# ohsnyt/bzip2-rust

Hardware: AMD Instinct MI355X
Metric: compress MB/s at -9 (900 KB blocks), 1/2/4/8 MI355X; bit-exact vs C bzip2 (higher is better)
Workload: dtype u8; 1 GPU; 1024 MiB per GPU synthetic text at -9 (1194 blocks on this rank), BASELINE configs[2]; raw_bytes_total=1073741824, blocks_rank0=1194, compressed_bytes=323302688

## Files before the change

bzip2-rust_amd/csrc/bzx_bsort.hip:

```cpp
#include <hip/hip_runtime.h>
#include "bzx_host.h"
#include "bzx_wg.h"
#include "bzx_pack.h"

#define BS_NT 1024
#define BS_NW (BS_NT / 64)
#ifndef BS_C
#define BS_C 2048
#endif
#define BS_FW (BS_C / 64)
#define BS_ISO (BS_C / 3)
#ifndef BS_ISO_SHIFT
#define BS_ISO_SHIFT 5
#endif
#ifndef BS_BIN1
#define BS_BIN1 15
#endif
#define BS_BIN2 12
#define BS_NBIN1 (1u << BS_BIN1)
#define BS_TAB_WORDS (BS_NBIN1 + (BS_NBIN1 >> 5))
#define BS_MAX_BK 1024
#ifndef BS_MAX_BIG
#define BS_MAX_BIG 512
#endif
#define SP_U 4
#ifndef BS_MAX_DEPTH
#define BS_MAX_DEPTH 511
#endif
#ifndef BS_MAX_SPLITS
#define BS_MAX_SPLITS 1024
#endif
#ifndef BS_ROUNDS
#define BS_ROUNDS 4
#endif
#ifndef BS_KEYBITS
#define BS_KEYBITS 32
#endif
#define BS_TINY 64
#define BS_MED 512
#define REC_IDX(r) ((uint32_t)((r) >> 12) & 0xFFFFFu)
#define REC_PREV(r) ((uint32_t)((r) >> 4) & 0xFFu)
#define W_POS_MASK 0x3FFFull

static_assert(BS_C <= 16384, "bucket capacity");

#ifdef BZX_DIAG
__shared__ unsigned long long s_diag[128];
#define DIAG_T0()                                                             \
    unsigned long long t_last_ = 0;                                           \
    if (B.dbg && threadIdx.x == 0) {                                          \
        for (int i_ = 0; i_ < 128; i_++) s_diag[i_] = 0;                      \
        t_last_ = wall_clock64();                                             \
    }                                                                         \
    (void)t_last_;
#define DIAG_STAMP(slot)                                                      \
    do {                                                                      \
        if (B.dbg && threadIdx.x == 0) {                                      \
            const unsigned long long now_ = wall_clock64();                   \
            s_diag[slot] += now_ - t_last_;                                   \
            t_last_ = now_;                                                   \
        }                                                                     \
    } while (0)
#define DIAG_COUNT(slot, v)                                                   \
    do {                                                                      \
        if (B.dbg && threadIdx.x == 0) s_diag[slot] += (unsigned long long)(v); \
    } while (0)
#define DIAG_FLUSH()                                                          \
    do {                                                                      \
        if (B.dbg && threadIdx.x == 0)                                        \
            for (int i_ = 0; i_ < 128; i_++)                                  \
                if (s_diag[i_]) atomicAdd(&B.dbg[i_], s_diag[i_]);            \
    } while (0)
#else
#define DIAG_T0() do {} while (0)
#define DIAG_STAMP(slot) do {} while (0)
#define DIAG_COUNT(slot, v) do {} while (0)
#define DIAG_FLUSH() do {} while (0)
#endif

__shared__ uint32_t b_tab[BS_TAB_WORDS + BS_MAX_BK];
__shared__ uint32_t b_start[BS_MAX_BK + 1];
__shared__ uint32_t b_first[BS_MAX_BK + 1];
__shared__ uint32_t b_cur[BS_MAX_BK];
__shared__ uint8_t b_b0[BS_MAX_BK];
__shared__ uint32_t b_inuse[256];
__shared__ uint8_t b_seq[256];
__shared__ uint32_t b_scratch[2 * BS_NW];
__shared__ uint32_t b_lbase[8];
__shared__ uint32_t b_bcast[12];
__shared__ uint32_t b_big[BS_MAX_BIG][3];

#define TAB(b) b_tab[(b) + ((b) >> 5)]

template <int ISO, int PER>
__device__ __forceinline__ void bucket_flags(const uint32_t (&c)[PER], uint32_t bin0, uint32_t excl, uint32_t prevc, uint32_t &fl, uint32_t &nf)
{
    constexpr uint32_t CP = BS_C - ISO;
    uint32_t s = excl, ps = excl - prevc, pc = prevc;
#pragma unroll
    for (int k = 0; k < PER; k++) {
        const bool f = (bin0 + k == 0) || c[k] > (uint32_t)ISO || pc > (uint32_t)ISO || (s / CP != ps / CP);
        fl |= (uint32_t)f << k;
        nf += f;
        ps = s;
        s += c[k];
        pc = c[k];
    }
}

template <int BINS, bool TAB16 = false>
__device__ __forceinline__ uint32_t form_buckets(uint32_t total)
{
    constexpr int PER = BINS / BS_NT;
    const uint32_t tid = threadIdx.x, bin0 = tid * PER;
    uint32_t c[PER], sum = 0, e8 = 0, e6 = 0, e4 = 0;
#pragma unroll
    for (int k = 0; k < PER; k++) {
        c[k] = TAB(bin0 + k);
        sum += c[k];
        const uint32_t m = c[k] <= BS_ISO ? c[k] : 0u;
        e8 += m > BS_C / 8 ? m : 0u;
        e6 += m > BS_C / 6 ? m : 0u;
        e4 += m > BS_C / 4 ? m : 0u;
    }
    const uint32_t prevc = tid ? TAB(bin0 - 1) : 0u;
    if (__any(e8 != 0)) {
        e8 = bzx_wave_incl_sum(e8);
        e6 = bzx_wave_incl_sum(e6);
        e4 = bzx_wave_incl_sum(e4);
        if (bzx_lane() == 63) {
            atomicAdd(&b_bcast[8], e8);
            if (e6) atomicAdd(&b_bcast[9], e6);
            if (e4) atomicAdd(&b_bcast[10], e4);
        }
    }
    uint32_t tot;
    const uint32_t excl = bzx_block_excl_sum<BS_NT>(sum, b_scratch, tot);
    const uint32_t allow = total >> BS_ISO_SHIFT;
    uint32_t fl = 0, nf = 0;
    if (b_bcast[8] <= allow) bucket_flags<BS_C / 8>(c, bin0, excl, prevc, fl, nf);
    else if (b_bcast[9] <= allow) bucket_flags<BS_C / 6>(c, bin0, excl, prevc, fl, nf);
    else if (b_bcast[10] <= allow) bucket_flags<BS_C / 4>(c, bin0, excl, prevc, fl, nf);
    else bucket_flags<BS_ISO>(c, bin0, excl, prevc, fl, nf);
    uint32_t nbk;
    const uint32_t fexcl = bzx_block_excl_sum<BS_NT>(nf, b_scratch, nbk);
    if (nbk > BS_MAX_BK) return 0;
    {
        uint32_t id = fexcl, s = excl;
#pragma unroll
        for (int k = 0; k < PER; k++) {
            if ((fl >> k) & 1u) {
                b_start[id] = s;
                b_first[id] = bin0 + k;
                id++;
            }
            if (TAB16) reinterpret_cast<uint16_t *>(b_tab)[bin0 + k] = (uint16_t)(id - 1);
            else TAB(bin0 + k) = id - 1;
            s += c[k];
        }
    }
    if (tid == 0) {
        b_start[nbk] = total;
        b_first[nbk] = BINS;
    }
    __syncthreads();
    return nbk;
}

template <int BINW>
__device__ __forceinline__ void bucket_setup(uint32_t nbk)
{
    for (uint32_t k = threadIdx.x; k < nbk; k += BS_NT) {
        const uint32_t first = b_first[k], last = b_first[k + 1] - 1u;
        b_b0[k] = (uint8_t)(first == last ? BINW : (uint32_t)__builtin_clz(first ^ last) - (32u - BINW));
        b_cur[k] = 0;
    }
}

template <int BINW>
__device__ __forceinline__ bool bucket_emit(const BzxBatch &B, uint32_t blk, uint32_t jj, uint32_t nbk, uint32_t base, uint32_t buf,
                                            uint32_t depth, uint32_t bits, uint32_t done, uint32_t salt)
{
    const uint32_t tid = threadIdx.x, cap8 = B.bk_cap >> 3;
    if (!B.bk_affine) jj += salt;
    if (tid < 8) {
        const uint32_t mine = B.bk_affine ? (tid == (jj & 7u) ? nbk : 0u) : (nbk + 7u - ((tid - jj) & 7u)) >> 3;
        uint32_t at = mine ? atomicAdd(&B.counters[BZX_CTR_BK_LIST0 + tid], mine) : 0u;
        if (at + mine > cap8) {
            b_bcast[4] = 1;
            at = 0;
        }
        b_lbase[tid] = tid * cap8 + at;
    }
    __syncthreads();
    if (b_bcast[4]) return false;
    for (uint32_t k = tid; k < nbk; k += BS_NT) {
        BzxBucket it;
        it.blk = blk;
        it.start = (base + b_start[k]) | (buf << 31);
        it.cnt = b_start[k + 1] - b_start[k];
        it.dbits = (depth + b_b0[k]) | (bits << 16);
        if (it.cnt > BS_C) {
            const uint32_t q = atomicAdd(&b_bcast[3], 1u);
            if (q - done < BS_MAX_BIG) {
                b_big[q % BS_MAX_BIG][0] = it.start;
                b_big[q % BS_MAX_BIG][1] = it.cnt;
                b_big[q % BS_MAX_BIG][2] = depth + BINW;
            } else {
                b_bcast[4] = 1;
            }
            it.cnt = 0;
        }
        B.bk_list[B.bk_affine ? b_lbase[jj & 7u] + k : b_lbase[(jj + k) & 7u] + (k >> 3)] = it;
    }
    __syncthreads();
    return b_bcast[4] == 0;
}

struct BzxDeepItem {
    uint32_t blk, st, cnt, dbits;
};

__device__ __forceinline__ uint32_t *rank_array(const BzxBatch &B, uint32_t k, uint32_t which)
{
    if (k >= B.rk_blocks) return nullptr;
    return B.isa2 + ((size_t)k * 2 + which) * BZX_MAX_N;
}

__device__ __forceinline__ void emit_giant(const BzxBatch &B, uint32_t blk, uint64_t *rec_a, const uint64_t *rec_b,
                                           uint32_t st, uint32_t cnt, uint32_t depth, uint32_t bits)
{
    const uint32_t tid = threadIdx.x, base = st & 0x7fffffffu;
    const uint64_t *src = ((st >> 31) ? rec_b : rec_a) + base;
    uint32_t *__restrict__ isa0 = rank_array(B, (uint32_t)BZX_SLAB(B, blk), 0), *__restrict__ isa1 = rank_array(B, (uint32_t)BZX_SLAB(B, blk), 1);
    if (tid == 0) b_bcast[7] = isa0 ? atomicAdd(&B.counters[BZX_CTR_GIANT_CNT], 1u) : 0xFFFFFFFFu;
    __syncthreads();
    const uint32_t at = b_bcast[7];
    const bool listed = at < B.deep_cap;
    for (uint32_t i = tid; i < cnt; i += BS_NT) {
        const uint64_t r = src[i];
        rec_a[base + i] = (uint64_t)REC_IDX(r) | (i == 0 ? 1ull << 32 : 0ull);
        if (isa0) isa0[REC_IDX(r)] = isa1[REC_IDX(r)] = base | (listed ? 0u : RK_COARSE);
    }
    if (tid == 0) {
        atomicMin(&B.blk[blk].n_mtf, depth / bits);
        if (listed) {
            BzxDeepItem it;
            it.blk = blk;
            it.st = base;
            it.cnt = cnt;
            it.dbits = 0;
            reinterpret_cast<BzxDeepItem *>(B.deep_list)[(size_t)2 * B.deep_cap + at] = it;
        }
        atomicAdd(&B.blk[blk].n_groups, 1u);
        if ((atomicOr(&B.blk[blk].status, BZX_ST_RESUME) & BZX_ST_RESUME) == 0)
            B.resume_list[atomicAdd(&B.counters[BZX_CTR_RESUME], 1u)] = blk;
    }
    __syncthreads();
}

__device__ __forceinline__ void block_redo(const BzxBatch &B, uint32_t b)
{
    if ((atomicOr(&B.blk[b].status, BZX_ST_REDO) & BZX_ST_REDO) == 0)
        B.redo_list[atomicAdd(&B.counters[BZX_CTR_REDO], 1u)] = b;
}


__device__ bool deep_process(const BzxBatch &B, uint32_t b, uint32_t j_, uint32_t n, uint32_t bits, const uint8_t *__restrict__ P,
                             uint64_t *__restrict__ rec_a, uint64_t *__restrict__ rec_b, uint32_t done, uint32_t flush_from,
                             int push_lvl)
{
    const uint32_t tid = threadIdx.x;
    bool ok = true;
    while (ok) {
        const uint32_t nbig = b_bcast[3];
        __syncthreads();
        if (done >= nbig) break;
        if (push_lvl >= 0 && done >= flush_from) {
            const uint32_t np = nbig - done;
            if (tid == 0) b_bcast[5] = atomicAdd(&B.counters[BZX_CTR_DEEP_CNT + push_lvl], np);
            __syncthreads();
            const uint32_t at = b_bcast[5];
            __syncthreads();
            if (at + np <= B.deep_cap) {
                BzxDeepItem *dl = reinterpret_cast<BzxDeepItem *>(B.deep_list) + (size_t)(push_lvl & 1) * B.deep_cap + at;
                for (uint32_t q = tid; q < np; q += BS_NT) {
                    const uint32_t r = (done + q) % BS_MAX_BIG;
                    BzxDeepItem it;
                    it.blk = b;
                    it.st = b_big[r][0];
                    it.cnt = b_big[r][1];
                    it.dbits = b_big[r][2] | (bits << 16);
                    dl[q] = it;
                }
                __syncthreads();
                break;
            }
            push_lvl = -1;
        }
        const uint32_t st = b_big[done % BS_MAX_BIG][0], cnt = b_big[done % BS_MAX_BIG][1], depth = b_big[done % BS_MAX_BIG][2];
        done++;
        if (tid == 0) b_bcast[6] = atomicAdd(reinterpret_cast<uint32_t *>(&B.blk[b].pack_word), 1u);
        __syncthreads();
        const uint32_t spent = b_bcast[6];
        const uint32_t base = st & 0x7fffffffu, buf = st >> 31;
        const uint64_t *__restrict__ src = (buf ? rec_b : rec_a) + base;
        uint64_t *__restrict__ dst = (buf ? rec_a : rec_b) + base;
        if (depth + BS_BIN2 + 32 >= n * bits) {
            ok = false;
            break;
        }
        if (depth + BS_BIN2 > BS_MAX_DEPTH || spent >= BS_MAX_SPLITS) {
            emit_giant(B, b, rec_a, rec_b, st, cnt, depth, bits);
            continue;
        }
        constexpr uint32_t NB2 = 1u << BS_BIN2;
        for (uint32_t i = tid; i < NB2 + (NB2 >> 5); i += BS_NT) b_tab[i] = 0;
        if (tid == 0) b_bcast[1] = 0;
        if (tid < 3) b_bcast[8 + tid] = 0;
        __syncthreads();
        for (uint32_t i = tid; i < cnt; i += BS_NT) atomicAdd(&TAB((uint32_t)(src[i] >> (64 - BS_BIN2))), 1u);
        __syncthreads();
        const uint32_t nbk = form_buckets<(int)NB2>(cnt);
        if (nbk == 0) {
            ok = false;
            break;
        }
        bucket_setup<BS_BIN2>(nbk);
        __syncthreads();
        for (uint32_t i = tid; i < cnt; i += BS_NT) {
            const uint64_t r = src[i];
            const uint32_t k = TAB((uint32_t)(r >> (64 - BS_BIN2)));
            uint32_t x = REC_IDX(r) * bits + depth + b_b0[k];
            if (x >= n * bits) x -= n * bits;
            const uint32_t key = (uint32_t)(pk_window_bit(P, x) >> 32);
            const uint32_t slot = atomicAdd(&b_cur[k], 1u);
            dst[b_start[k] + slot] = ((uint64_t)key << 32) | (r & 0xFFFFFFFFull);
        }
        __syncthreads();
        ok = bucket_emit<BS_BIN2>(B, b, j_, nbk, base, buf ^ 1u, depth, bits, done, spent + 1u);
        DIAG_COUNT(104, 1);
        DIAG_COUNT(105, cnt);
    }
    return ok;
}

__global__ __launch_bounds__(BS_NT) void bzx_bsplit_kernel(BzxBatch B)
{
    const uint32_t tid = threadIdx.x;
    DIAG_T0();
    for (;;) {
        if (tid == 0) b_bcast[0] = atomicAdd(&B.counters[BZX_CTR_SPLIT_FETCH], 1u);
        __syncthreads();
        const uint32_t j_ = b_bcast[0];
        __syncthreads();
        if (j_ >= B.nblk) break;
        const uint32_t b = B.blk_first + j_ * B.blk_step;
        const uint32_t n = B.blk[b].n;
        const uint8_t *__restrict__ T = BZX_BLOCK_PTR(B, B.blk[b]);
        const size_t sb = BZX_SLAB(B, b);
        uint8_t *__restrict__ P = B.pk + sb * BZX_PK_STRIDE;
        uint64_t *__restrict__ rec_a = B.rec_a + sb * BZX_MAX_N;
        uint64_t *__restrict__ rec_b = B.rec_b + sb * BZX_MAX_N;

        DIAG_STAMP(96);
        if (tid < 256) b_inuse[tid] = 0;
        if (tid == 0) {
            b_bcast[1] = 0;
            b_bcast[3] = 0;
            b_bcast[4] = 0;
            b_bcast[8] = b_bcast[9] = b_bcast[10] = 0;
            B.blk[b].pack_word = 0;
            B.blk[b].n_mtf = 0xFFFFFFFFu;
            B.blk[b].n_groups = 0;
            B.blk[b].n_selectors = (uint32_t)BZX_SLAB(B, b);
        }
        __syncthreads();
        {
            const uint32_t n16 = n & ~15u;
            for (uint32_t i = tid * 16; i < n16; i += BS_NT * 16) {
                uint4 v;
                __builtin_memcpy(&v, T + i, 16);
                const uint32_t w[4] = {v.x, v.y, v.z, v.w};
#pragma unroll
                for (int q = 0; q < 4; q++)
#pragma unroll
                    for (int k = 0; k < 4; k++) b_inuse[(w[q] >> (8 * k)) & 255u] = 1;
            }
            for (uint32_t i = n16 + tid; i < n; i += BS_NT) b_inuse[T[i]] = 1;
        }
        __syncthreads();
        uint32_t n_in_use;
        {
            const uint32_t flag = tid < 256 ? b_inuse[tid] : 0u;
            const uint32_t ex = bzx_block_excl_sum<BS_NT>(flag, b_scratch, n_in_use);
            if (tid < 256) b_seq[tid] = (uint8_t)ex;
        }
        __syncthreads();
        uint32_t bits = 1;
        while ((1u << bits) < n_in_use) bits++;
        DIAG_STAMP(97);
        pk_build_t<BS_NT>(T, n, bits, P, b_seq);
        DIAG_STAMP(98);

        for (uint32_t i = tid; i < BS_TAB_WORDS; i += BS_NT) b_tab[i] = 0;
        __syncthreads();
        for (uint32_t t0 = 0; t0 < n; t0 += BS_NT * 4 * SP_U) {
            uint64_t x[SP_U];
#pragma unroll
            for (uint32_t u = 0; u < SP_U; u++) {
                const uint32_t i0 = t0 + (u * BS_NT + tid) * 4;
                x[u] = i0 < n ? pk_window(P, i0, bits) : 0ull;
            }
#pragma unroll
            for (uint32_t u = 0; u < SP_U; u++) {
                const uint32_t i0 = t0 + (u * BS_NT + tid) * 4;
#pragma unroll
                for (uint32_t e = 0; e < 4; e++)
                    if (i0 + e < n) atomicAdd(&TAB((uint32_t)((x[u] << (e * bits)) >> (64 - BS_BIN1))), 1u);
            }
        }
        __syncthreads();
        DIAG_STAMP(99);
        uint32_t nbk = form_buckets<(int)BS_NBIN1, true>(n);
        if (nbk) bucket_setup<BS_BIN1>(nbk);
        __syncthreads();
        DIAG_STAMP(100);
        if (nbk == 0) {
            DIAG_COUNT(106, 1);
            if (tid == 0) block_redo(B, b);
            __syncthreads();
            continue;
        }

        {
            constexpr uint32_t SP_TILE = 8192, SP_V = SP_TILE / (BS_NT * 4);
            static_assert(BS_MAX_BK <= BS_NT && BS_TAB_WORDS >= 32768 + BS_MAX_BK, "tile scan: one bucket per lane");
            uint16_t *tab16 = reinterpret_cast<uint16_t *>(b_tab);
            for (uint32_t i = tid; i < BS_NBIN1 / 2; i += BS_NT) {
                uint32_t v = reinterpret_cast<uint32_t *>(b_tab)[i];
                v |= ((uint32_t)b_b0[v & 1023u] << 10) | ((uint32_t)b_b0[(v >> 16) & 1023u] << 26);
                reinterpret_cast<uint32_t *>(b_tab)[i] = v;
            }
            uint64_t *stage = reinterpret_cast<uint64_t *>(b_tab + 16384);
            uint32_t *tcnt0 = b_tab + 32768;
            uint32_t *delta = b_first;
            uint32_t *tcnt1 = tcnt0 + BS_MAX_BK;
            if (tid < nbk) tcnt0[tid] = tcnt1[tid] = 0;
            uint64_t hi[SP_V], lo[SP_V];
            uint32_t pv[SP_V];
            auto load_tile = [&](uint32_t t0) {
#pragma unroll
                for (uint32_t u = 0; u < SP_V; u++) {
                    const uint32_t i0 = t0 + (u * BS_NT + tid) * 4;
                    hi[u] = lo[u] = 0;
                    pv[u] = 0;
                    if (i0 < n) {
                        uint64_t w2[2];
                        __builtin_memcpy(w2, P + ((i0 * bits) >> 3), 16);
                        hi[u] = w2[0];
                        lo[u] = w2[1];
                        if (i0 >= 1 && i0 + 3 <= n) {
                            __builtin_memcpy(&pv[u], T + i0 - 1, 4);
                        } else {
                            const uint32_t nvalid = n - i0 < 4u ? n - i0 : 4u;
                            for (uint32_t e = 0; e < nvalid; e++) pv[u] |= (uint32_t)T[i0 + e ? i0 + e - 1 : n - 1] << (8 * e);
                        }
                    }
                }
            };
            load_tile(0);
            bzx_lds_barrier();
            uint32_t tpar = 0;
            for (uint32_t t0 = 0; t0 < n; t0 += SP_TILE, tpar ^= 1u) {
                uint32_t *tcnt = tpar ? tcnt1 : tcnt0, *tother = tpar ? tcnt0 : tcnt1;
                uint32_t kr[SP_V * 4], key[SP_V * 4], pvc[SP_V];
#pragma unroll
                for (uint32_t u = 0; u < SP_V; u++) {
                    const uint32_t i0 = t0 + (u * BS_NT + tid) * 4;
                    const uint32_t nvalid = i0 < n ? (n - i0 < 4u ? n - i0 : 4u) : 0u;
                    const uint32_t sh0 = (i0 * bits) & 7u;
                    const uint64_t h = __builtin_bswap64(hi[u]), l = __builtin_bswap64(lo[u]);
                    pvc[u] = pv[u];
#pragma unroll
                    for (uint32_t e = 0; e < 4; e++) {
                        kr[u * 4 + e] = 0xFFFFFFFFu;
                        key[u * 4 + e] = 0;
                        if (e < nvalid) {
                            const uint32_t sh = sh0 + e * bits;
                            const uint64_t w = sh ? (h << sh) | (l >> (64u - sh)) : h;
                            const uint32_t kb = tab16[(uint32_t)(w >> (64 - BS_BIN1))], k = kb & 1023u;
                            key[u * 4 + e] = (uint32_t)((w << (kb >> 10)) >> 32);
                            kr[u * 4 + e] = k | (atomicAdd(&tcnt[k], 1u) << 16);
                        }
                    }
                }
                if (t0 + SP_TILE < n) load_tile(t0 + SP_TILE);
                bzx_lds_barrier();
                {
                    const uint32_t c = tid < nbk ? tcnt[tid] : 0u;
                    const uint32_t incl = bzx_wave_incl_sum(c);
                    uint32_t *wtot = b_scratch + tpar * BS_NW;
                    if (bzx_lane() == 63) wtot[bzx_wave()] = incl;
                    bzx_lds_barrier();
                    uint32_t pre = 0;
                    const uint32_t wv = bzx_wave();
#pragma unroll
                    for (uint32_t i = 0; i < BS_NW; i++) pre += i < wv ? wtot[i] : 0u;
                    const uint32_t ex = pre + incl - c;
                    if (tid < nbk) {
                        tcnt[tid] = ex;
                        tother[tid] = 0;
                        delta[tid] = b_start[tid] + b_cur[tid] - ex;
                        b_cur[tid] += c;
                    }
                }
                bzx_lds_barrier();
#pragma unroll
                for (uint32_t u = 0; u < SP_V; u++)
#pragma unroll
                    for (uint32_t e = 0; e < 4; e++)
                        if (kr[u * 4 + e] != 0xFFFFFFFFu) {
                            const uint32_t k = kr[u * 4 + e] & 0xFFFFu, rel = (u * BS_NT + tid) * 4 + e;
                            stage[tcnt[k] + (kr[u * 4 + e] >> 16)] = ((uint64_t)key[u * 4 + e] << 32) | ((uint64_t)k << 21) | ((uint64_t)rel << 8) |
                                                                     (uint64_t)((pvc[u] >> (8 * e)) & 255u);
                        }
                bzx_lds_barrier();
                const uint32_t tn = n - t0 < SP_TILE ? n - t0 : SP_TILE;
#pragma unroll
                for (uint32_t u = 0; u < SP_TILE / BS_NT; u++) {
                    const uint32_t i = u * BS_NT + tid;
                    if (i < tn) {
                        const uint64_t r = stage[i];
                        const uint32_t k = (uint32_t)(r >> 21) & 1023u, rel = (uint32_t)(r >> 8) & 8191u;
                        rec_a[delta[k] + i] = (r & 0xFFFFFFFF00000000ull) | ((uint64_t)(t0 + rel) << 12) | ((r & 255ull) << 4);
                    }
                }
            }
        }
        __syncthreads();
        DIAG_STAMP(101);
        bool ok = bucket_emit<BS_BIN1>(B, b, j_, nbk, 0, 0, 0, bits, 0, 0);
        DIAG_STAMP(102);

        if (ok) ok = deep_process(B, b, j_, n, bits, P, rec_a, rec_b, 0, 0, BZX_DEEP_LEVELS > 0 ? 0 : -1);
        DIAG_STAMP(103);
        if (!ok) DIAG_COUNT(107, 1);
        if (!ok && tid == 0) block_redo(B, b);
        __syncthreads();
    }
    DIAG_FLUSH();
}

__global__ __launch_bounds__(BS_NT) void bzx_bsplit_deep_kernel(BzxBatch B)
{
    const uint32_t tid = threadIdx.x, lvl = B.deep_lvl;
    const uint32_t listed = B.counters[BZX_CTR_DEEP_CNT + lvl];
    const uint32_t n_items = listed < B.deep_cap ? listed : B.deep_cap;
    if (n_items == 0) return;
    DIAG_T0();
    const BzxDeepItem *list = reinterpret_cast<const BzxDeepItem *>(B.deep_list) + (size_t)(lvl & 1u) * B.deep_cap;
    for (;;) {
        if (tid == 0) b_bcast[0] = atomicAdd(&B.counters[BZX_CTR_DEEP_FETCH + lvl], 1u);
        __syncthreads();
        const uint32_t i = b_bcast[0];
        __syncthreads();
        if (i >= n_items) break;
        const BzxDeepItem d = list[i];
        if (d.cnt == 0) continue;
        const uint32_t b = d.blk;
        if (__atomic_load_n(&B.blk[b].status, __ATOMIC_RELAXED) & BZX_ST_REDO) continue;
        const uint32_t n = B.blk[b].n, bits = d.dbits >> 16;
        const size_t sb = BZX_SLAB(B, b);
        const uint8_t *__restrict__ P = B.pk + sb * BZX_PK_STRIDE;
        uint64_t *__restrict__ rec_a = B.rec_a + sb * BZX_MAX_N;
        uint64_t *__restrict__ rec_b = B.rec_b + sb * BZX_MAX_N;
        if (tid == 0) {
            b_bcast[3] = 1;
            b_bcast[4] = 0;
            b_big[0][0] = d.st;
            b_big[0][1] = d.cnt;
            b_big[0][2] = d.dbits & 0xFFFFu;
        }
        __syncthreads();
        const bool ok = deep_process(B, b, (b - B.blk_first) / B.blk_step, n, bits, P, rec_a, rec_b, 0, 1,
                                     lvl + 1 < BZX_DEEP_LEVELS ? (int)lvl + 1 : -1);
        if (!ok && tid == 0) block_redo(B, b);
        __syncthreads();
    }
    DIAG_FLUSH();
}

#ifndef SK_NT
#define SK_NT 256
#endif
#define SK_NW (SK_NT / 64)
#define BS_E (BS_C / SK_NT)
#define SK_DB 8
#define SK_ND (1u << SK_DB)
static_assert(BS_C % SK_NT == 0 && BS_E >= 1 && BS_E <= 8, "bucket capacity");

__shared__ uint64_t s_x[BS_C];
__shared__ __attribute__((aligned(16))) uint64_t s_w[BS_C + 4];
__shared__ __attribute__((aligned(16))) uint32_t s_cnt[SK_NW][SK_ND];
__shared__ uint32_t s_dbase[SK_ND];
__shared__ uint32_t s_part[4];
__shared__ uint64_t s_f[BS_FW + 1];
__shared__ uint32_t s_med[BS_C / BS_TINY + 1];
__shared__ uint32_t s_large[BS_C / BS_MED + 1];
__shared__ uint32_t s_rc[2][4];
__shared__ uint32_t s_bc[8];
__shared__ uint32_t s_m[2];
__shared__ uint32_t s_red[SK_NW][4];

__device__ __forceinline__ uint32_t uni(uint32_t v) { return bzx_uni(v); }
__device__ __forceinline__ uint32_t tid_here() { return bzx_tid_here(); }
__device__ __forceinline__ BzxBucket uni(BzxBucket b)
{
    BzxBucket r;
    r.blk = uni(b.blk);
    r.start = uni(b.start);
    r.cnt = uni(b.cnt);
    if (r.cnt >> 31) r.cnt = 0;
    r.dbits = uni(b.dbits);
    return r;
}

__device__ __forceinline__ void wave_rank(uint32_t *wc, uint32_t d, bool valid, uint32_t lane, uint32_t &old, uint32_t &rank)
{
    uint64_t m = __ballot(valid);
    uint32_t plo = (uint32_t)m, phi = (uint32_t)(m >> 32);
#pragma unroll
    for (int b = 0; b < SK_DB; b++) {
        const uint32_t mask = 0u - ((d >> b) & 1u);
        m = __ballot((d >> b) & 1u);
        plo &= ~((uint32_t)m ^ mask);
        phi &= ~((uint32_t)(m >> 32) ^ mask);
    }
    const uint64_t peers = ((uint64_t)phi << 32) | plo;
    rank = (uint32_t)__popcll(peers & ((1ull << lane) - 1ull));
    old = wc[d];
    lds_order();
    if (valid && rank == 0) atomicAdd(&wc[d], (uint32_t)__popcll(peers));
    lds_order();
}

__device__ __attribute__((noinline)) void wg_radix_sort(uint32_t base, uint32_t cnt, int lo, int hi)
{
    uint64_t *A = s_w + base;
    const uint32_t tid = threadIdx.x, lane = bzx_lane(), wave = bzx_wave();
    const uint32_t rows = (cnt + SK_NT - 1) / SK_NT, chunk = rows * 64;
    if (tid == 0) {
        s_bc[5] = 0;
        s_bc[6] = 0;
    }
    __syncthreads();
    {
        const uint64_t a0 = A[0];
        uint64_t d = 0;
#pragma unroll
        for (uint32_t j = 0; j < BS_E; j++) {
            const uint32_t e = wave * chunk + j * 64 + lane;
            if (j < rows && e < cnt) d |= A[e] ^ a0;
        }
#pragma unroll
        for (int s = 32; s > 0; s >>= 1) d |= __shfl_xor(d, s);
        if (lane == 0 && d) {
            atomicOr(&s_bc[5], (uint32_t)d);
            atomicOr(&s_bc[6], (uint32_t)(d >> 32));
        }
    }
    __syncthreads();
    const uint64_t diff = ((uint64_t)s_bc[6] << 32) | s_bc[5];
    uint32_t *wc = s_cnt[wave];
    for (int shift = lo; shift < hi; shift += SK_DB) {
        if (((diff >> shift) & (uint64_t)(SK_ND - 1)) == 0) continue;
#pragma unroll
        for (uint32_t i = 0; i < SK_ND / 64; i++) wc[i * 64 + lane] = 0;
        lds_order();
        uint64_t v[BS_E];
        uint32_t old[BS_E], rk[BS_E];
#pragma unroll
        for (uint32_t j = 0; j < BS_E; j++) {
            const uint32_t e = wave * chunk + j * 64 + lane;
            v[j] = j < rows && e < cnt ? A[e] : 0ull;
        }
#pragma unroll
        for (uint32_t j = 0; j < BS_E; j++) {
            const uint32_t e = wave * chunk + j * 64 + lane;
            wave_rank(wc, (uint32_t)(v[j] >> shift) & (SK_ND - 1), j < rows && e < cnt, lane, old[j], rk[j]);
        }
        __syncthreads();
        {
            constexpr uint32_t SK_DK = SK_ND > SK_NT ? SK_ND / SK_NT : 1u;
            if (tid * SK_DK < SK_ND) {
                uint32_t tot[SK_DK], sum = 0;
#pragma unroll
                for (uint32_t i = 0; i < SK_DK; i++) {
                    uint32_t run = 0;
#pragma unroll
                    for (int w = 0; w < SK_NW; w++) {
                        const uint32_t t = s_cnt[w][tid * SK_DK + i];
                        s_cnt[w][tid * SK_DK + i] = run;
                        run += t;
                    }
                    tot[i] = run;
                    sum += run;
                }
                const uint32_t incl = bzx_wave_incl_sum(sum);
                uint32_t run = incl - sum;
#pragma unroll
                for (uint32_t i = 0; i < SK_DK; i++) {
                    s_dbase[tid * SK_DK + i] = run;
                    run += tot[i];
                }
                if (lane == 63) s_part[wave] = incl;
            }
        }
        __syncthreads();
        const uint32_t p1 = s_part[0], p2 = p1 + s_part[1], p3 = p2 + s_part[2];
#pragma unroll
        for (uint32_t j = 0; j < BS_E; j++) {
            const uint32_t e = wave * chunk + j * 64 + lane;
            if (j < rows && e < cnt) {
                const uint32_t d = (uint32_t)(v[j] >> shift) & (SK_ND - 1);
                const uint32_t q = SK_ND > SK_NT ? 0u : d >> 6;
                A[s_dbase[d] + (q == 0 ? 0u : q == 1 ? p1 : q == 2 ? p2 : p3) + wc[d] + old[j] + rk[j]] = v[j];
            }
        }
        __syncthreads();
    }
}

__device__ __attribute__((noinline)) void wg_radix_sort_opt(uint32_t cnt, int lo, int hi)
{
    uint64_t *A = s_x;
    const uint32_t lane = bzx_lane(), wave = bzx_wave();
    const uint32_t rows = (cnt + SK_NT - 1) / SK_NT, chunk = rows * 64;
    __syncthreads();
    uint64_t diff;
    {
        uint32_t o0 = 0, o1 = 0, a0 = ~0u, a1 = ~0u;
#pragma unroll
        for (int w = 0; w < SK_NW; w++) {
            o0 |= s_red[w][0];
            o1 |= s_red[w][1];
            a0 &= s_red[w][2];
            a1 &= s_red[w][3];
        }
        diff = ((uint64_t)(o1 & ~a1) << 32) | (o0 & ~a0);
    }
    uint32_t *wc = s_cnt[wave];
    uint32_t *wb = reinterpret_cast<uint32_t *>(s_w) + wave * SK_ND;
    for (int shift = lo; shift < hi; shift += SK_DB) {
        if (((diff >> shift) & (uint64_t)(SK_ND - 1)) == 0) continue;
#pragma unroll
        for (uint32_t i = 0; i < SK_ND / 64; i++) wc[i * 64 + lane] = 0;
        lds_order();
        uint64_t v[BS_E];
        uint32_t old[BS_E];
#pragma unroll
        for (uint32_t j = 0; j < BS_E; j++) {
            const uint32_t e = wave * chunk + j * 64 + lane;
            v[j] = j < rows && e < cnt ? A[e] : 0ull;
        }
#pragma unroll
        for (uint32_t j = 0; j < BS_E; j++) {
            const uint32_t e = wave * chunk + j * 64 + lane;
            old[j] = bzx_lds_ticket(&wc[(uint32_t)(v[j] >> shift) & (SK_ND - 1)], j < rows && e < cnt);
        }
        __syncthreads();
        {
            static_assert(SK_ND == 4 * 64, "four digits per lane");
            uint32_t mine[4], tot[4], sum = 0;
#pragma unroll
            for (uint32_t i = 0; i < 4; i++) mine[i] = tot[i] = 0;
#pragma unroll
            for (uint32_t w = 0; w < SK_NW; w++) {
                const uint4 c = *reinterpret_cast<const uint4 *>(&s_cnt[w][4 * lane]);
                const uint32_t cc[4] = {c.x, c.y, c.z, c.w};
#pragma unroll
                for (uint32_t i = 0; i < 4; i++) {
                    if (w < wave) mine[i] += cc[i];
                    tot[i] += cc[i];
                }
            }
#pragma unroll
            for (uint32_t i = 0; i < 4; i++) sum += tot[i];
            uint32_t run = bzx_wave_incl_sum(sum) - sum;
            uint4 o;
            o.x = run + mine[0];
            run += tot[0];
            o.y = run + mine[1];
            run += tot[1];
            o.z = run + mine[2];
            run += tot[2];
            o.w = run + mine[3];
            *reinterpret_cast<uint4 *>(&wb[4 * lane]) = o;
        }
        lds_order();
#pragma unroll
        for (uint32_t j = 0; j < BS_E; j++) {
            const uint32_t e = wave * chunk + j * 64 + lane;
            if (j < rows && e < cnt) A[wb[(uint32_t)(v[j] >> shift) & (SK_ND - 1)] + old[j]] = v[j];
        }
        __syncthreads();
    }
}

template <bool TICKETS>
__device__ __attribute__((noinline)) void wave_radix_sort(uint32_t base, uint32_t s, int lo, int hi)
{
    constexpr uint32_t ROWS = BS_MED / 64;
    uint64_t *A = s_w + base;
    uint32_t *wc = s_cnt[bzx_wave()];
    const uint32_t lane = bzx_lane();
    const uint32_t rows = (s + 63u) / 64u;
    uint64_t v[ROWS];
    uint64_t diff = 0;
    {
        const uint64_t a0 = A[0];
#pragma unroll
        for (uint32_t j = 0; j < ROWS; j++) {
            const uint32_t e = j * 64 + lane;
            v[j] = e < s ? A[e] : 0ull;
            if (e < s) diff |= v[j] ^ a0;
        }
#pragma unroll
        for (int sh = 32; sh > 0; sh >>= 1) diff |= __shfl_xor(diff, sh);
    }
    for (int shift = lo; shift < hi; shift += SK_DB) {
        if (((diff >> shift) & (uint64_t)(SK_ND - 1)) == 0) continue;
#pragma unroll
        for (uint32_t i = 0; i < SK_ND / 64; i++) wc[i * 64 + lane] = 0;
        lds_order();
        uint32_t old[ROWS], rk[ROWS];
#pragma unroll
        for (uint32_t j = 0; j < ROWS; j++) {
            old[j] = rk[j] = 0;
            if (j < rows) {
                if (TICKETS) old[j] = bzx_lds_ticket(&wc[(uint32_t)(v[j] >> shift) & (SK_ND - 1)], j * 64 + lane < s);
                else wave_rank(wc, (uint32_t)(v[j] >> shift) & (SK_ND - 1), j * 64 + lane < s, lane, old[j], rk[j]);
            }
        }
        {
            uint32_t c[SK_ND / 64], sum = 0;
#pragma unroll
            for (uint32_t i = 0; i < SK_ND / 64; i++) {
// ... 1205 lines not shown
```

Baseline: 32590 MB/s.

## Replace 16-bit bin table with compact popcount bucket table and enlarge scatter tile

Replaces the per-bin 16-bit bucket/shift table with a compact per-32-bin (prefix, flag-word) pair, where the bucket is recovered by popcount and the shift is read from b_b0. This removes the pass that rewrote the whole table and frees LDS. The freed space holds a larger staging tile (12288 entries instead of 8192), so fewer tile iterations and barriers are needed per block. The record packing widens the rel field to 14 bits, and deep_process is force-inlined. The costs are an extra popcount and an extra LDS lookup per key, plus higher register pressure from inlining.

```diff
diff --git a/bzip2-rust_amd/csrc/bzx_bsort.hip b/bzip2-rust_amd/csrc/bzx_bsort.hip
--- a/bzip2-rust_amd/csrc/bzx_bsort.hip
+++ b/bzip2-rust_amd/csrc/bzx_bsort.hip
@@ -24,6 +24,9 @@
 #define BS_MAX_BIG 512
 #endif
 #define SP_U 4
+#ifndef BS_SP_TILE
+#define BS_SP_TILE 12288
+#endif
 #ifndef BS_MAX_DEPTH
 #define BS_MAX_DEPTH 511
 #endif
@@ -38,6 +41,11 @@
 #endif
 #define BS_TINY 64
 #define BS_MED 512
+#ifdef BZX_HIP_EMU
+#define BS_INLINE_CALL
+#else
+#define BS_INLINE_CALL [[clang::always_inline]]
+#endif
 #define REC_IDX(r) ((uint32_t)((r) >> 12) & 0xFFFFFu)
 #define REC_PREV(r) ((uint32_t)((r) >> 4) & 0xFFu)
 #define W_POS_MASK 0x3FFFull
@@ -78,7 +86,7 @@
 #define DIAG_FLUSH() do {} while (0)
 #endif
 
-__shared__ uint32_t b_tab[BS_TAB_WORDS + BS_MAX_BK];
+__shared__ __attribute__((aligned(16))) uint32_t b_tab[BS_TAB_WORDS + BS_MAX_BK];
 __shared__ uint32_t b_start[BS_MAX_BK + 1];
 __shared__ uint32_t b_first[BS_MAX_BK + 1];
 __shared__ uint32_t b_cur[BS_MAX_BK];
@@ -92,6 +100,11 @@
 
 #define TAB(b) b_tab[(b) + ((b) >> 5)]
 
+__device__ __forceinline__ uint32_t ctab_bucket(uint2 p, uint32_t bin)
+{
+    return p.x + (uint32_t)__popc(p.y & ((2u << (bin & 31u)) - 1u)) - 1u;
+}
+
 template <int ISO, int PER>
 __device__ __forceinline__ void bucket_flags(const uint32_t (&c)[PER], uint32_t bin0, uint32_t excl, uint32_t prevc, uint32_t &fl, uint32_t &nf)
 {
@@ -108,10 +121,11 @@
     }
 }
 
-template <int BINS, bool TAB16 = false>
+template <int BINS, bool CTAB = false>
 __device__ __forceinline__ uint32_t form_buckets(uint32_t total)
 {
     constexpr int PER = BINS / BS_NT;
+    static_assert(!CTAB || PER == 32, "compact table: one flag word per lane");
     const uint32_t tid = threadIdx.x, bin0 = tid * PER;
     uint32_t c[PER], sum = 0, e8 = 0, e6 = 0, e4 = 0;
 #pragma unroll
@@ -154,10 +168,10 @@
                 b_first[id] = bin0 + k;
                 id++;
             }
-            if (TAB16) reinterpret_cast<uint16_t *>(b_tab)[bin0 + k] = (uint16_t)(id - 1);
-            else TAB(bin0 + k) = id - 1;
+            if (!CTAB) TAB(bin0 + k) = id - 1;
             s += c[k];
         }
+        if (CTAB) reinterpret_cast<uint2 *>(b_tab)[tid] = make_uint2(fexcl, fl);
     }
     if (tid == 0) {
         b_start[nbk] = total;
@@ -434,16 +448,14 @@
         }
 
         {
-            constexpr uint32_t SP_TILE = 8192, SP_V = SP_TILE / (BS_NT * 4);
-            static_assert(BS_MAX_BK <= BS_NT && BS_TAB_WORDS >= 32768 + BS_MAX_BK, "tile scan: one bucket per lane");
-            uint16_t *tab16 = reinterpret_cast<uint16_t *>(b_tab);
-            for (uint32_t i = tid; i < BS_NBIN1 / 2; i += BS_NT) {
-                uint32_t v = reinterpret_cast<uint32_t *>(b_tab)[i];
-                v |= ((uint32_t)b_b0[v & 1023u] << 10) | ((uint32_t)b_b0[(v >> 16) & 1023u] << 26);
-                reinterpret_cast<uint32_t *>(b_tab)[i] = v;
-            }
-            uint64_t *stage = reinterpret_cast<uint64_t *>(b_tab + 16384);
-            uint32_t *tcnt0 = b_tab + 32768;
+            constexpr uint32_t SP_TILE = BS_SP_TILE, SP_V = SP_TILE / (BS_NT * 4);
+            constexpr uint32_t SP_REL = 14;
+            static_assert(SP_V >= 1 && SP_V * BS_NT * 4 == SP_TILE && SP_TILE <= (1u << SP_REL), "tile: whole groups per lane, place in SP_REL bits");
+            static_assert(BS_MAX_BK <= BS_NT && BS_MAX_BK <= (1u << (24 - SP_REL)), "tile scan: one bucket per lane; bucket in the entry's top bits");
+            static_assert(2 * BS_NT + 2 * BS_MAX_BK + 2 * SP_TILE <= BS_TAB_WORDS + BS_MAX_BK, "table, counts and parking area inside b_tab");
+            const uint2 *ctab = reinterpret_cast<const uint2 *>(b_tab);
+            uint32_t *tcnt0 = b_tab + 2 * BS_NT;
+            uint64_t *stage = reinterpret_cast<uint64_t *>(b_tab + 2 * BS_NT + 2 * BS_MAX_BK);
             uint32_t *delta = b_first;
             uint32_t *tcnt1 = tcnt0 + BS_MAX_BK;
             if (tid < nbk) tcnt0[tid] = tcnt1[tid] = 0;
@@ -489,8 +501,8 @@
                         if (e < nvalid) {
                             const uint32_t sh = sh0 + e * bits;
                             const uint64_t w = sh ? (h << sh) | (l >> (64u - sh)) : h;
-                            const uint32_t kb = tab16[(uint32_t)(w >> (64 - BS_BIN1))], k = kb & 1023u;
-                            key[u * 4 + e] = (uint32_t)((w << (kb >> 10)) >> 32);
+                            const uint32_t bin = (uint32_t)(w >> (64 - BS_BIN1)), k = ctab_bucket(ctab[bin >> 5], bin);
+                            key[u * 4 + e] = (uint32_t)((w << b_b0[k]) >> 32);
                             kr[u * 4 + e] = k | (atomicAdd(&tcnt[k], 1u) << 16);
                         }
                     }
@@ -522,17 +534,17 @@
                     for (uint32_t e = 0; e < 4; e++)
                         if (kr[u * 4 + e] != 0xFFFFFFFFu) {
                             const uint32_t k = kr[u * 4 + e] & 0xFFFFu, rel = (u * BS_NT + tid) * 4 + e;
-                            stage[tcnt[k] + (kr[u * 4 + e] >> 16)] = ((uint64_t)key[u * 4 + e] << 32) | ((uint64_t)k << 21) | ((uint64_t)rel << 8) |
+                            stage[tcnt[k] + (kr[u * 4 + e] >> 16)] = ((uint64_t)key[u * 4 + e] << 32) | ((uint64_t)k << (8 + SP_REL)) | ((uint64_t)rel << 8) |
                                                                      (uint64_t)((pvc[u] >> (8 * e)) & 255u);
                         }
                 bzx_lds_barrier();
                 const uint32_t tn = n - t0 < SP_TILE ? n - t0 : SP_TILE;
-#pragma unroll
+#pragma unroll 4
                 for (uint32_t u = 0; u < SP_TILE / BS_NT; u++) {
                     const uint32_t i = u * BS_NT + tid;
                     if (i < tn) {
                         const uint64_t r = stage[i];
-                        const uint32_t k = (uint32_t)(r >> 21) & 1023u, rel = (uint32_t)(r >> 8) & 8191u;
+                        const uint32_t k = (uint32_t)(r >> (8 + SP_REL)) & 1023u, rel = (uint32_t)(r >> 8) & ((1u << SP_REL) - 1u);
                         rec_a[delta[k] + i] = (r & 0xFFFFFFFF00000000ull) | ((uint64_t)(t0 + rel) << 12) | ((r & 255ull) << 4);
                     }
                 }
@@ -543,7 +555,7 @@
         bool ok = bucket_emit<BS_BIN1>(B, b, j_, nbk, 0, 0, 0, bits, 0, 0);
         DIAG_STAMP(102);
 
-        if (ok) ok = deep_process(B, b, j_, n, bits, P, rec_a, rec_b, 0, 0, BZX_DEEP_LEVELS > 0 ? 0 : -1);
+        if (ok) BS_INLINE_CALL ok = deep_process(B, b, j_, n, bits, P, rec_a, rec_b, 0, 0, BZX_DEEP_LEVELS > 0 ? 0 : -1);
         DIAG_STAMP(103);
         if (!ok) DIAG_COUNT(107, 1);
         if (!ok && tid == 0) block_redo(B, b);
```

Result: no change. 32920 MB/s, median of 6 (+1.0%).
